# ramanathanlab/distllm

Measured on NVIDIA H100. Metric: embedded chunks/sec @512-tok, higher is better.
Workload: dtype bf16

## Files before the change

### distllm_b200/csrc/attention.cuh

```cuda
#pragma once

#include "common.cuh"

namespace b2e {

constexpr int AT_KC = 64;
constexpr float AT_MASKED = -3.0e38f;

template <int D, int V>
struct AtCfg {
  static constexpr int COLS = D < 64 ? D : 64;
  static constexpr int ROW_BYTES = 2 * COLS;
  static constexpr int BOX = 64 * ROW_BYTES;
  static constexpr int NB = D / COLS;
  static constexpr int NWG = (V & 64) ? 4 : 2;
  static constexpr int QT = 64 * NWG;
  static constexpr int THREADS = 128 * NWG + (NWG == 4 ? 128 : 32);
  static constexpr int CONSUMER_REGS = 112, PRODUCER_REGS = 24;
  static constexpr int STAGES = D == 128 ? 3 : 4;
  static constexpr int Q_BYTES = NWG * NB * BOX;
  static constexpr int STAGE_BYTES = 2 * NB * BOX;
  static_assert(D == 32 || D == 64 || D == 128, "head_dim");
  static constexpr int BAR = Q_BYTES + STAGES * STAGE_BYTES;
  static constexpr int SMEM_BYTES = BAR + 256 + 1024;
  static_assert(SMEM_BYTES <= 232448, "shared memory");
};

__device__ long long* g_att_clock = nullptr;

__device__ __forceinline__ float poly_exp2(float x) {
  x = fmaxf(x, -126.0f);
  const float n = rintf(x);
  const float f = x - n;
  float p = fmaf(f, 9.6181291e-3f, 5.5504109e-2f);
  p = fmaf(f, p, 2.4022651e-1f);
  p = fmaf(f, p, 6.9314718e-1f);
  p = fmaf(f, p, 1.0f);
  return __int_as_float(__float_as_int(p) + (static_cast<int>(n) << 23));
}

template <int ROW_BYTES>
__device__ __forceinline__ uint64_t at_box_desc(uint32_t saddr) {
  if constexpr (ROW_BYTES == 128) return make_smem_desc_sw128(saddr);
  else return make_smem_desc_sw64(saddr);
}

__global__ void attn_prep_kernel(const int64_t* __restrict__ mask, float* __restrict__ bias,
                                 int* __restrict__ kv_chunks, int* __restrict__ plain_chunks, int B, int S,
                                 int S_pad) {
  const int b = blockIdx.x * (blockDim.x >> 5) + (threadIdx.x >> 5);
  if (b >= B) return;
  const int lane = threadIdx.x & 31;
  int last = 0;
  int first_off = S_pad;
  for (int j = lane; j < S_pad; j += 32) {
    float v = -INFINITY;
    bool on = false;
    if (j < S) {
      on = mask[static_cast<size_t>(b) * S + j] != 0;
      v = on ? 0.0f : AT_MASKED;
      if (on) last = j + 1;
    }
    if (!on) first_off = min(first_off, j);
    bias[static_cast<size_t>(b) * S_pad + j] = v;
  }
#pragma unroll
  for (int o = 16; o > 0; o >>= 1) {
    last = max(last, __shfl_xor_sync(0xffffffffu, last, o));
    first_off = min(first_off, __shfl_xor_sync(0xffffffffu, first_off, o));
  }
  if (lane == 0) {
    kv_chunks[b] = last > 0 ? (last + AT_KC - 1) / AT_KC : S_pad / AT_KC;
    plain_chunks[b] = first_off / AT_KC;
  }
}

template <int D, int MODE, int V>
__global__ void __launch_bounds__(AtCfg<D, V>::THREADS, 1)
attention_kernel(const __grid_constant__ CUtensorMap tm, const __grid_constant__ CUtensorMap tm_ctx,
                 const float* __restrict__ bias, const int* __restrict__ kv_chunks,
                 const int* __restrict__ plain_chunks, int B, int S, int S_pad, int heads, int kv_heads, int window,
                 float scale_log2e, const int* __restrict__ seq_cu, const int* __restrict__ seq_len,
                 h16* __restrict__ ctx) {
  using Cfg = AtCfg<D, V>;
  constexpr int NB = Cfg::NB;
  constexpr int COLS = Cfg::COLS, BOX = Cfg::BOX, RB = Cfg::ROW_BYTES;
  constexpr int NWG = Cfg::NWG;
  constexpr int POLY = (V >> 2) & 3;
  constexpr bool EPI_ROLE = (V & 128) != 0;
  constexpr bool STAMPS = (V & 256) != 0;
  static_assert(MODE == 0 || (V & ~(64 | 128)) == 0, "windowed / causal attention: warpgroups and epilogue role only");
  const int h = blockIdx.x % heads;
  const int b = (blockIdx.x / heads) % B;
  const int tile = static_cast<int>(gridDim.x / (heads * B)) - 1 - static_cast<int>(blockIdx.x / (heads * B));
  const int row0 = seq_cu != nullptr ? __ldg(seq_cu + b) : b * S;
  const int len = seq_len != nullptr ? __ldg(seq_len + b) : S;
  const int q0 = tile * Cfg::QT;
  if (q0 >= len) return;
  const int kvc = __ldg(kv_chunks + b);
  const int np = (V & 1) ? __ldg(plain_chunks + b) : 0;
  int lo = 0, hi = kvc;
  if (MODE == 1) {
    lo = max(0, q0 - window) / AT_KC;
    hi = min(kvc, (q0 + Cfg::QT - 1 + window) / AT_KC + 1);
  } else if (MODE == 2) {
    lo = window > 0 ? max(0, q0 - window + 1) / AT_KC : 0;
    hi = min(kvc, (q0 + Cfg::QT - 1) / AT_KC + 1);
  }
  if (lo >= hi) lo = hi - 1;

  extern __shared__ uint8_t smem_raw[];
  const uint32_t sb = (smem_u32(smem_raw) + 1023u) & ~1023u;
  const uint32_t q_bar = sb + Cfg::BAR;
  const uint32_t full_bar = q_bar + 8;
  const uint32_t empty_bar = full_bar + 8u * Cfg::STAGES;
  const uint32_t out_bar = empty_bar + 8u * Cfg::STAGES;
  const int warp = threadIdx.x >> 5;
  const int kvh = h / (heads / kv_heads);
  const int qcol = h * D, kcol = (heads + kvh) * D, vcol = (heads + kv_heads + kvh) * D;

  if (threadIdx.x == 0) {
    mbar_init(q_bar, 1);
    for (int s = 0; s < Cfg::STAGES; ++s) {
      mbar_init(full_bar + 8u * s, 1);
      mbar_init(empty_bar + 8u * s, NWG);
    }
    for (int w = 0; w < NWG; ++w) mbar_init(out_bar + 8u * w, 1);
    mbar_fence_init();
  }
  __syncthreads();

  if (warp >= 4 * NWG) {
    if constexpr (NWG == 4) asm volatile("setmaxnreg.dec.sync.aligned.u32 %0;" ::"n"(Cfg::PRODUCER_REGS));
    if (warp == 4 * NWG && elect_one()) {
      tma_prefetch_desc(&tm);
      mbar_expect_tx(q_bar, Cfg::Q_BYTES);
#pragma unroll
      for (int w = 0; w < NWG; ++w)
#pragma unroll
        for (int x = 0; x < NB; ++x)
          tma_load_2d(sb + (w * NB + x) * BOX, &tm, q_bar, qcol + COLS * x, row0 + q0 + 64 * w);
      int stage = 0;
      uint32_t phase = 0;
      for (int c = lo; c < hi; ++c) {
        mbar_wait(empty_bar + 8u * stage, phase ^ 1u);
        const uint32_t fb = full_bar + 8u * stage;
        const uint32_t dst = sb + Cfg::Q_BYTES + stage * Cfg::STAGE_BYTES;
        mbar_expect_tx(fb, Cfg::STAGE_BYTES);
#pragma unroll
        for (int x = 0; x < NB; ++x) {
          tma_load_2d(dst + x * BOX, &tm, fb, kcol + COLS * x, row0 + c * AT_KC);
          tma_load_2d(dst + (NB + x) * BOX, &tm, fb, vcol + COLS * x, row0 + c * AT_KC);
        }
        if (++stage == Cfg::STAGES) { stage = 0; phase ^= 1u; }
      }
      if constexpr (EPI_ROLE) {
        for (int w = 0; w < NWG; ++w) {
          mbar_wait(out_bar + 8u * w, 0);
          if (q0 + 64 * w + 64 > len) continue;
#pragma unroll
          for (int x = 0; x < NB; ++x)
            tma_store_2d(&tm_ctx, sb + (w * NB + x) * BOX, h * D + COLS * x, row0 + q0 + 64 * w);
        }
        tma_store_commit();
        tma_store_wait_all();
      }
    }
    return;
  }

  if constexpr (NWG == 4) asm volatile("setmaxnreg.inc.sync.aligned.u32 %0;" ::"n"(Cfg::CONSUMER_REGS));
  const int wg = warp >> 2;
  const int t = threadIdx.x & 127;
  const int quad = t & 3;
  const int qr = q0 + 64 * wg + 16 * (t >> 5) + ((t & 31) >> 2);
  const float* brow = bias + static_cast<size_t>(b) * S_pad;
  const uint32_t q_addr = sb + wg * NB * BOX;
  long long* clk = nullptr;
  int n_stamp = 0;
  if (STAMPS && blockIdx.x == 0 && threadIdx.x == 0) clk = g_att_clock;

  constexpr int OG = COLS / 8;
  float o[NB][4 * OG];
#pragma unroll
  for (int x = 0; x < NB; ++x)
#pragma unroll
    for (int i = 0; i < 4 * OG; ++i) o[x][i] = 0.0f;
  float m[2] = {-INFINITY, -INFINITY}, l[2] = {0.0f, 0.0f};

  mbar_wait(q_bar, 0);
  int stage = 0;
  uint32_t phase = 0;
  for (int c = lo; c < hi; ++c) {
    mbar_wait(full_bar + 8u * stage, phase);
    const uint32_t k_addr = sb + Cfg::Q_BYTES + stage * Cfg::STAGE_BYTES;
    const uint32_t v_addr = k_addr + NB * BOX;
    float s[32];
#pragma unroll
    for (int i = 0; i < 32; ++i) s[i] = 0.0f;
    wgmma_fence();
    constexpr int KB = COLS / 16;
#pragma unroll
    for (int kk = 0; kk < D / 16; ++kk)
      wgmma_64x64_ss<0>(s, at_box_desc<RB>(q_addr + (kk / KB) * BOX) + 2u * (kk % KB),
                        at_box_desc<RB>(k_addr + (kk / KB) * BOX) + 2u * (kk % KB), kk != 0);
    wgmma_commit();
    wgmma_wait<0>();
    reg_fence(s);
    if (STAMPS && clk != nullptr && n_stamp < 256) {
      clk[n_stamp] = clock64();
      clk[256 + n_stamp++] = 2 * c + 1;
    }

    const int kbase = c * AT_KC + 2 * quad;
    const bool plain = MODE == 0 && (V & 1) && c < np;
#pragma unroll
    for (int j = 0; j < 8; ++j) {
      const float2 bz = plain ? make_float2(0.0f, 0.0f) : *reinterpret_cast<const float2*>(brow + kbase + 8 * j);
#pragma unroll
      for (int e = 0; e < 4; ++e) {
        const int key = kbase + 8 * j + (e & 1);
        const int q = qr + 8 * (e >> 1);
        float x = fmaf(s[4 * j + e], scale_log2e, (e & 1) ? bz.y : bz.x);
        if (MODE == 1 && abs(q - key) > window) x = AT_MASKED;
        if (MODE == 2 && (key > q || (window > 0 && q - key >= window))) x = AT_MASKED;
        s[4 * j + e] = x;
      }
    }
    float alpha[2];
#pragma unroll
    for (int hf = 0; hf < 2; ++hf) {
      float mx = m[hf];
#pragma unroll
      for (int j = 0; j < 8; ++j) mx = fmaxf(mx, fmaxf(s[4 * j + 2 * hf], s[4 * j + 2 * hf + 1]));
      mx = fmaxf(mx, __shfl_xor_sync(0xffffffffu, mx, 1));
      mx = fmaxf(mx, __shfl_xor_sync(0xffffffffu, mx, 2));
      alpha[hf] = fast_exp2(m[hf] - mx);
      m[hf] = mx;
    }
    uint32_t p[4][4];
    float rs[2] = {0.0f, 0.0f};
#pragma unroll
    for (int j = 0; j < 8; ++j) {
#pragma unroll
      for (int hf = 0; hf < 2; ++hf) {
        const float x0 = s[4 * j + 2 * hf] - m[hf], x1 = s[4 * j + 2 * hf + 1] - m[hf];
        const int k0 = (2 * (j & 1) + hf) * 2;
        const float p0 = (k0 % 4) < POLY ? poly_exp2(x0) : fast_exp2(x0);
        const float p1 = ((k0 + 1) % 4) < POLY ? poly_exp2(x1) : fast_exp2(x1);
        rs[hf] += p0 + p1;
        p[j >> 1][(j & 1) * 2 + hf] = pack_h16x2(p0, p1);
      }
    }
#pragma unroll
    for (int hf = 0; hf < 2; ++hf) l[hf] = l[hf] * alpha[hf] + rs[hf];
#pragma unroll
    for (int x = 0; x < NB; ++x)
#pragma unroll
      for (int j = 0; j < OG; ++j) {
        o[x][4 * j + 0] *= alpha[0];
        o[x][4 * j + 1] *= alpha[0];
        o[x][4 * j + 2] *= alpha[1];
        o[x][4 * j + 3] *= alpha[1];
      }

#pragma unroll
    for (int x = 0; x < NB; ++x) reg_fence(o[x]);
    wgmma_fence();
#pragma unroll
    for (int kc = 0; kc < 4; ++kc)
#pragma unroll
      for (int x = 0; x < NB; ++x) {
        if constexpr (COLS == 64) wgmma_64x64_rs_tb(o[x], p[kc], make_smem_desc_sw128(v_addr + x * BOX + kc * 16 * 128));
        else wgmma_64x32_rs_tb(o[x], p[kc], make_smem_desc_sw64(v_addr + x * BOX + kc * 16 * 64));
      }
    wgmma_commit();
    wgmma_wait<0>();
#pragma unroll
    for (int x = 0; x < NB; ++x) reg_fence(o[x]);
    if (STAMPS && clk != nullptr && n_stamp < 256) {
      clk[n_stamp] = clock64();
      clk[256 + n_stamp++] = 2 * c + 2;
    }
    if (t == 0) mbar_arrive(empty_bar + 8u * stage);
    if (++stage == Cfg::STAGES) { stage = 0; phase ^= 1u; }
  }

  const bool staged = EPI_ROLE && q0 + 64 * wg + 64 <= len;
#pragma unroll
  for (int hf = 0; hf < 2; ++hf) {
    float tot = l[hf];
    tot += __shfl_xor_sync(0xffffffffu, tot, 1);
    tot += __shfl_xor_sync(0xffffffffu, tot, 2);
    const float inv = 1.0f / tot;
    const int q = qr + 8 * hf;
    if (staged) {
      const int r = q - q0 - 64 * wg;
      const int swz = RB == 128 ? (r & 7) : ((r >> 1) & 3);
#pragma unroll
      for (int x = 0; x < NB; ++x)
#pragma unroll
        for (int j = 0; j < OG; ++j) {
          const uint32_t off = r * RB + ((j ^ swz) << 4) + 4 * quad;
          *reinterpret_cast<uint32_t*>(smem_raw + (q_addr - smem_u32(smem_raw)) + x * BOX + off) =
              pack_h16x2(o[x][4 * j + 2 * hf] * inv, o[x][4 * j + 2 * hf + 1] * inv);
        }
      continue;
    }
    if (q >= len) continue;
    h16* orow = ctx + static_cast<size_t>(row0 + q) * (heads * D) + h * D + 2 * quad;
#pragma unroll
    for (int x = 0; x < NB; ++x)
#pragma unroll
      for (int j = 0; j < OG; ++j)
        *reinterpret_cast<uint32_t*>(orow + COLS * x + 8 * j) =
            pack_h16x2(o[x][4 * j + 2 * hf] * inv, o[x][4 * j + 2 * hf + 1] * inv);
  }
  if constexpr (EPI_ROLE) {
    fence_proxy_async_smem();
    asm volatile("bar.sync %0, 128;" ::"r"(1 + wg) : "memory");
    if (t == 0) mbar_arrive(out_bar + 8u * wg);
  }
}

}
```

### distllm_b200/csrc/b2e_api.cu

```cuda
#include "../../include/b2e.h"
#include "../../include/b2e_debug.h"

#include <cuda.h>
#include <cuda_runtime.h>

#include <cstdarg>
#include <cstdio>
#include <cstdlib>
#include <cstring>
#include <string>
#include <utility>
#include <vector>

#include "attention.cuh"
#include "binsearch.cuh"
#include "common.cuh"
#include "gemm.cuh"
#include "mistral_ops.cuh"
#include "pack.cuh"
#include "rowops.cuh"
#include "topk.cuh"
#include "topk_tc.cuh"

using namespace b2e;
// ... 102 lines not shown
  info->ok = true;
  return B2E_OK;
}

int current_device_info(DeviceInfo* info) {
  int dev = 0;
  if (cudaGetDevice(&dev) != cudaSuccess) {
    cudaGetLastError();
    return fail(B2E_ERR_NO_DEVICE, "no CUDA device visible; libb2e has no CPU fallback");
  }
  static DeviceInfo cache[64];
  if (dev < 64 && cache[dev].ok) {
    *info = cache[dev];
    return B2E_OK;
  }
  int rc = device_info(dev, info);
  if (rc == B2E_OK && dev < 64) cache[dev] = *info;
  return rc;
}

template <typename Kern>
int ensure_smem_attr(Kern kern, int bytes) {
  static std::vector<std::pair<const void*, int>> done;
  int dev = 0;
  CUDA_TRY(cudaGetDevice(&dev));
  const void* key = reinterpret_cast<const void*>(kern);
  for (const auto& d : done)
    if (d.first == key && d.second == dev) return B2E_OK;
  CUDA_TRY(cudaFuncSetAttribute(kern, cudaFuncAttributeMaxDynamicSharedMemorySize, bytes));
  done.emplace_back(key, dev);
  return B2E_OK;
}

int check_gemm_shape(int M, int N, int K) {
  if (M <= 0 || N <= 0 || K <= 0) return fail(B2E_ERR_INVALID, "gemm: empty shape %dx%dx%d", M, N, K);
  if (N % 128 != 0) return fail(B2E_ERR_INVALID, "gemm: N=%d must be a multiple of 128", N);
  if (K % 64 != 0) return fail(B2E_ERR_INVALID, "gemm: K=%d must be a multiple of 64", K);
  return B2E_OK;
}

bool g_gemm_profiling = false;

template <int EPI>
int launch_gemm_epi(const CUtensorMap& ta, const CUtensorMap& tb, void* out, const float* bias,
                    const h16* resid, int M, int N, int K, cudaStream_t st, const int* m_dev) {
  auto kern = gemm_h16_wgmma_kernel<EPI>;
  if constexpr (EPI == EPI_BIAS)
    if (g_gemm_profiling) kern = gemm_h16_wgmma_kernel<EPI, true>;
  int rc = ensure_smem_attr(kern, GEMM_SMEM_BYTES);
  if (rc) return rc;
  DeviceInfo dev;
  if ((rc = current_device_info(&dev))) return rc;
  const long long tiles = (long long)(N / GEMM_BN) * ((M + GEMM_BM - 1) / GEMM_BM);
  if (tiles > 0x7fffffffLL) return fail(B2E_ERR_INVALID, "gemm: %lld output tiles exceed one grid", tiles);
  CUtensorMap tm_out;
  if ((rc = make_tmap_h16(&tm_out, out, M, epi_is_glu(EPI) ? N / 2 : N, GEMM_BM))) return rc;
  const unsigned grid = (unsigned)(tiles < dev.sms ? tiles : dev.sms);
  kern<<<grid, GEMM_THREADS, GEMM_SMEM_BYTES, st>>>(ta, tb, tm_out, static_cast<h16*>(out), bias, resid, M, N, K,
                                                    m_dev);
  CUDA_TRY(cudaGetLastError());
  return B2E_OK;
}

int launch_gemm(const CUtensorMap& ta, const CUtensorMap& tb, void* out, const float* bias,
                const void* resid, int M, int N, int K, int epi, cudaStream_t st, const int* m_dev = nullptr) {
  const h16* r = static_cast<const h16*>(resid);
  switch (epi) {
    case B2E_EPI_BIAS: return launch_gemm_epi<EPI_BIAS>(ta, tb, out, bias, r, M, N, K, st, m_dev);
    case B2E_EPI_BIAS_GELU: return launch_gemm_epi<EPI_BIAS_GELU>(ta, tb, out, bias, r, M, N, K, st, m_dev);
    case B2E_EPI_BIAS_RESID: return launch_gemm_epi<EPI_BIAS_RESID>(ta, tb, out, bias, r, M, N, K, st, m_dev);
    case B2E_EPI_SWIGLU: return launch_gemm_epi<EPI_SWIGLU>(ta, tb, out, bias, r, M, N, K, st, m_dev);
    case B2E_EPI_GEGLU: return launch_gemm_epi<EPI_GEGLU>(ta, tb, out, bias, r, M, N, K, st, m_dev);
  }
  return fail(B2E_ERR_INVALID, "unknown epilogue %d", epi);
}

struct AttnScratch {
  float* bias = nullptr;
  int* kv_chunks = nullptr;
  int* plain_chunks = nullptr;
  size_t cap_bias = 0, cap_b = 0;
  uint64_t gen = 0;
  int device = -1;
  int ensure(int B, int S_pad) {
    int dev = 0;
    CUDA_TRY(cudaGetDevice(&dev));
    if (dev != device) {
      release();
      device = dev;
      ++gen;
    }
    if ((size_t)B * S_pad > cap_bias || (size_t)B > cap_b) ++gen;
    if ((size_t)B * S_pad > cap_bias) {
      cudaFree(bias);
      bias = nullptr;
      cap_bias = 0;
      CUDA_TRY(cudaMalloc(&bias, sizeof(float) * (size_t)B * S_pad));
      cap_bias = (size_t)B * S_pad;
    }
    if ((size_t)B > cap_b) {
      cudaFree(kv_chunks); cudaFree(plain_chunks);
      kv_chunks = plain_chunks = nullptr;
      cap_b = 0;
      CUDA_TRY(cudaMalloc(&kv_chunks, sizeof(int) * B));
      CUDA_TRY(cudaMalloc(&plain_chunks, sizeof(int) * B));
      cap_b = B;
    }
    return B2E_OK;
  }
  void release() {
    cudaFree(bias); cudaFree(kv_chunks); cudaFree(plain_chunks);
    bias = nullptr; kv_chunks = plain_chunks = nullptr; cap_bias = cap_b = 0;
  }
};

inline int attn_s_pad(int S) { return (S + AT_KC - 1) / AT_KC * AT_KC; }

int attention_prepare(AttnScratch& sc, const int64_t* mask, int B, int S, cudaStream_t st) {
  int rc;
  const int S_pad = attn_s_pad(S);
  if ((rc = sc.ensure(B, S_pad))) return rc;
  attn_prep_kernel<<<(B + 7) / 8, 256, 0, st>>>(mask, sc.bias, sc.kv_chunks, sc.plain_chunks, B, S, S_pad);
  CUDA_TRY(cudaGetLastError());
  return B2E_OK;
}

struct SeqLayout {
  const int* cu = nullptr;
  const int* len = nullptr;
  const int* t_real = nullptr;
  const int* tok_src = nullptr;
};

template <int D, int MODE, int V>
int launch_attention_kernel(const CUtensorMap& tm, const AttnScratch& sc, void* ctx, int B, int S, int heads,
                            int kv_heads, int window, cudaStream_t st, const SeqLayout& lay) {
  using Cfg = AtCfg<D, V>;
  auto kern = attention_kernel<D, MODE, V>;
  int rc = ensure_smem_attr(kern, Cfg::SMEM_BYTES);
  if (rc) return rc;
  CUtensorMap tm_ctx = {};
  if ((V & 128) && (rc = make_tmap_h16(&tm_ctx, ctx, (uint64_t)B * S, (uint64_t)heads * D, 64, Cfg::COLS))) return rc;
  const float scale_log2e = 1.4426950408889634f / sqrtf(static_cast<float>(D));
  const long long ctas = (long long)heads * B * ((S + Cfg::QT - 1) / Cfg::QT);
  if (ctas > 0x7fffffffLL)
    return fail(B2E_ERR_INVALID, "attention: %lld CTAs (heads=%d B=%d S=%d) exceed one grid", ctas, heads, B, S);
  kern<<<(unsigned)ctas, Cfg::THREADS, Cfg::SMEM_BYTES, st>>>(tm, tm_ctx, sc.bias, sc.kv_chunks, sc.plain_chunks, B, S,
                                                    attn_s_pad(S), heads, kv_heads, window, scale_log2e, lay.cu,
                                                    lay.len, static_cast<h16*>(ctx));
  CUDA_TRY(cudaGetLastError());
  return B2E_OK;
}

constexpr int AT_DEFAULT_VARIANT = 193;
int g_att3_variant = -1;
inline int att3_variant() {
  if (g_att3_variant < 0) {
    const char* e = getenv("B2E_ATT3");
    g_att3_variant = e ? atoi(e) : AT_DEFAULT_VARIANT;
  }
  return g_att3_variant;
}

int launch_attention(const CUtensorMap& tkv, const AttnScratch& sc, void* ctx, int B, int S, int heads,
                     cudaStream_t st, int window = 0, const SeqLayout& lay = SeqLayout()) {
  const int v = att3_variant();
#define B2E_ATT(MODE, V) launch_attention_kernel<64, MODE, V>(tkv, sc, ctx, B, S, heads, heads, window, st, lay)
  if (window > 0) {
    switch (v & 192) {
      case 0: return B2E_ATT(1, 0);
      case 64: return B2E_ATT(1, 64);
      case 128: return B2E_ATT(1, 128);
      case 192: return B2E_ATT(1, 192);
    }
    return fail(B2E_ERR_INVALID, "windowed attention: variant %d has no instantiation (bits 6-7 of the variant pick "
                "0, 64, 128 or 192)", v);
  }
  switch (v) {
    case 0: return B2E_ATT(0, 0);
    case 1: return B2E_ATT(0, 1);
    case 5: return B2E_ATT(0, 5);
    case 64: return B2E_ATT(0, 64);
    case 65: return B2E_ATT(0, 65);
    case 69: return B2E_ATT(0, 69);
    case 193: return B2E_ATT(0, 193);
    case 261: return B2E_ATT(0, 261);
    case 321: return B2E_ATT(0, 321);
  }
#undef B2E_ATT
  return fail(B2E_ERR_INVALID, "attention variant %d is not instantiated (0,1,5,64,65,69,193,261,321)", v);
}

int launch_attention_causal_d128(const void* qkv, AttnScratch& sc, void* ctx, int B, int S, int heads,
                                 int kv_heads, int window, cudaStream_t st, const SeqLayout& lay = SeqLayout()) {
  CUtensorMap tm;
  const int rc = make_tmap_h16(&tm, qkv, (uint64_t)B * S, (uint64_t)(heads + 2 * kv_heads) * 128, AT_KC);
  if (rc) return rc;
  return launch_attention_kernel<128, 2, 0>(tm, sc, ctx, B, S, heads, kv_heads, window, st, lay);
}

constexpr int AT_D32_VARIANT = 1;

int launch_attention_bidir(const CUtensorMap& tqkv, const AttnScratch& sc, void* ctx, int B, int S, int heads,
                           int head_dim, cudaStream_t st, const SeqLayout& lay = SeqLayout()) {
  if (head_dim == 32)
    return launch_attention_kernel<32, 0, AT_D32_VARIANT>(tqkv, sc, ctx, B, S, heads, heads, 0, st, lay);
  return launch_attention(tqkv, sc, ctx, B, S, heads, st, 0, lay);
}

#define DISPATCH_H(H, CALL)                                         \
  switch (H) {                                                      \
    case 256: { constexpr int HW = 256; CALL; break; }              \
    case 384: { constexpr int HW = 384; CALL; break; }              \
    case 512: { constexpr int HW = 512; CALL; break; }              \
    case 640: { constexpr int HW = 640; CALL; break; }              \
    case 768: { constexpr int HW = 768; CALL; break; }              \
    case 1024: { constexpr int HW = 1024; CALL; break; }            \
    case 1280: { constexpr int HW = 1280; CALL; break; }            \
    case 2048: { constexpr int HW = 2048; CALL; break; }            \
    case 2560: { constexpr int HW = 2560; CALL; break; }            \
    case 4096: { constexpr int HW = 4096; CALL; break; }            \
    default: return fail(B2E_ERR_INVALID, "hidden size %d not supported (need 256*{1,2,3,4,5,8,10,16}, 384 or 640)", (H)); \
  }

inline int row_blocks(int rows) { return (rows + ROW_WARPS - 1) / ROW_WARPS; }

int check_h(int H) {
  if (H == 384 || H == 640) return B2E_OK;
  if (H % 256 != 0) return fail(B2E_ERR_INVALID, "hidden size %d must be a multiple of 256, or 384 or 640", H);
  switch (H / 256) {
    case 1: case 2: case 3: case 4: case 5: case 8: case 10: case 16: return B2E_OK;
  }
  return fail(B2E_ERR_UNSUPPORTED, "hidden size %d not supported (built: 256 x {1,2,3,4,5,8,10,16}, 384, 640)", H);
}

struct PoolScratch {
  int* seq_len = nullptr;
  int* kill = nullptr;
  int* idx = nullptr;
  float* w = nullptr;
  float* count = nullptr;
  float* part = nullptr;
  size_t cap_b = 0, cap_s = 0, cap_bs = 0, cap_part = 0;
  int device = -1;
  uint64_t gen = 0;

  int ensure(int B, int S, size_t part_elems) {
    int dev = 0;
    CUDA_TRY(cudaGetDevice(&dev));
    if (dev != device) {
      release();
      device = dev;
      ++gen;
    }
    if ((size_t)B > cap_b || (size_t)S > cap_s || (size_t)B * S > cap_bs || part_elems > cap_part) ++gen;
    if ((size_t)B > cap_b) {
      cudaFree(seq_len); cudaFree(idx); cudaFree(count);
      seq_len = idx = nullptr;
      count = nullptr;
      cap_b = 0;
      CUDA_TRY(cudaMalloc(&seq_len, sizeof(int) * B));
      CUDA_TRY(cudaMalloc(&idx, sizeof(int) * B));
      CUDA_TRY(cudaMalloc(&count, sizeof(float) * B));
      cap_b = B;
    }
    if ((size_t)S > cap_s) {
      cudaFree(kill);
      kill = nullptr;
      cap_s = 0;
      CUDA_TRY(cudaMalloc(&kill, sizeof(int) * S));
      cap_s = S;
    }
    if ((size_t)B * S > cap_bs) {
      cudaFree(w);
      w = nullptr;
      cap_bs = 0;
      CUDA_TRY(cudaMalloc(&w, sizeof(float) * (size_t)B * S));
      cap_bs = (size_t)B * S;
    }
    if (part_elems > cap_part) {
      cudaFree(part);
      part = nullptr;
      cap_part = 0;
      CUDA_TRY(cudaMalloc(&part, sizeof(float) * part_elems));
      cap_part = part_elems;
    }
    return B2E_OK;
  }
  void release() {
    cudaFree(seq_len); cudaFree(kill); cudaFree(idx); cudaFree(w); cudaFree(count); cudaFree(part);
    seq_len = kill = idx = nullptr; w = count = part = nullptr;
    cap_b = cap_s = cap_bs = cap_part = 0;
  }
};

inline int pool_nsplit(int S) {
  int n = (S + 63) / 64;
  return n < 1 ? 1 : (n > 16 ? 16 : n);
}

int launch_pool_weights(PoolScratch& ps, int64_t* mask, int B, int S, int pool_kind, int mutate,
                        cudaStream_t st) {
  seq_len_kernel<<<(B + 7) / 8, 256, 0, st>>>(mask, ps.seq_len, B, S);
  CUDA_TRY(cudaMemsetAsync(ps.kill, 0, sizeof(int) * S, st));
  kill_columns_kernel<<<(B + 255) / 256, 256, 0, st>>>(ps.seq_len, ps.kill, B, S);
  pool_weights_kernel<<<(B + 7) / 8, 256, 0, st>>>(mask, ps.seq_len, ps.kill, ps.w, ps.count, B, S,
                                                    pool_kind == B2E_POOL_MEAN_REF ? 1 : 0, mutate);
  CUDA_TRY(cudaGetLastError());
  return B2E_OK;
}

int launch_finalize(PoolScratch& ps, float* out, int B, int H, int nsplit, int l2, int round_mode,
                    cudaStream_t st) {
  pool_finalize_kernel<<<B, 256, (H + 32) * sizeof(float), st>>>(ps.part, ps.count, out, H, nsplit,
                                                                 l2, round_mode);
  CUDA_TRY(cudaGetLastError());
  return B2E_OK;
}

struct DeviceGuard {
  int prev = -1;
  DeviceGuard() {
    if (cudaGetDevice(&prev) != cudaSuccess) {
      cudaGetLastError();
      prev = -1;
    }
  }
  ~DeviceGuard() {
    if (prev >= 0) cudaSetDevice(prev);
  }
};

thread_local PoolScratch g_pool_scratch;
thread_local AttnScratch g_attn_scratch;

}

struct B2EEncoder {
  B2EModelDesc desc;
  int full_layers = 0;
  std::vector<const void*> w;
  int device = 0;
  int sms = 0;
// ... 1343 lines not shown
```

Baseline: 3170.

## Add persistent bidirectional attention kernel with double-buffered Q and TMA output stores

Adds a persistent attention kernel for head_dim 64 that loops over (head, batch, q-tile) work items on a grid sized to SM occupancy. Q is double-buffered so the producer can load the next tile's Q and K/V while consumers finish the current one, and the output is staged in the Q buffer and written with TMA stores. The default variant switches from 193 to 577, a 4-warpgroup persistent configuration. This is meant to cut per-CTA launch, prologue and epilogue cost and keep the pipeline full across tiles, at the price of doubling Q shared memory and a more complex barrier protocol.

```diff
diff --git a/distllm_b200/csrc/attention.cuh b/distllm_b200/csrc/attention.cuh
--- a/distllm_b200/csrc/attention.cuh
+++ b/distllm_b200/csrc/attention.cuh
@@ -19,9 +19,10 @@
   static constexpr int CONSUMER_REGS = 112, PRODUCER_REGS = 24;
   static constexpr int STAGES = D == 128 ? 3 : 4;
   static constexpr int Q_BYTES = NWG * NB * BOX;
+  static constexpr int Q_BUFS = (V & 512) ? 2 : 1;
   static constexpr int STAGE_BYTES = 2 * NB * BOX;
   static_assert(D == 32 || D == 64 || D == 128, "head_dim");
-  static constexpr int BAR = Q_BYTES + STAGES * STAGE_BYTES;
+  static constexpr int BAR = Q_BUFS * Q_BYTES + STAGES * STAGE_BYTES;
   static constexpr int SMEM_BYTES = BAR + 256 + 1024;
   static_assert(SMEM_BYTES <= 232448, "shared memory");
 };
@@ -323,4 +324,282 @@
   }
 }
 
-}
+
+__device__ __forceinline__ void at_softmax_chunk(float (&s)[32], float (&m)[2], float (&l)[2], float (&alpha)[2],
+                                                 const float* brow, int c, bool plain, int quad, float scale_log2e) {
+  const int kbase = c * AT_KC + 2 * quad;
+#pragma unroll
+  for (int j = 0; j < 8; ++j) {
+    const float2 bz = plain ? make_float2(0.0f, 0.0f) : *reinterpret_cast<const float2*>(brow + kbase + 8 * j);
+#pragma unroll
+    for (int e = 0; e < 4; ++e) s[4 * j + e] = fmaf(s[4 * j + e], scale_log2e, (e & 1) ? bz.y : bz.x);
+  }
+#pragma unroll
+  for (int hf = 0; hf < 2; ++hf) {
+    float mx = m[hf];
+#pragma unroll
+    for (int j = 0; j < 8; ++j) mx = fmaxf(mx, fmaxf(s[4 * j + 2 * hf], s[4 * j + 2 * hf + 1]));
+    mx = fmaxf(mx, __shfl_xor_sync(0xffffffffu, mx, 1));
+    mx = fmaxf(mx, __shfl_xor_sync(0xffffffffu, mx, 2));
+    alpha[hf] = fast_exp2(m[hf] - mx);
+    m[hf] = mx;
+  }
+  float rs[2] = {0.0f, 0.0f};
+#pragma unroll
+  for (int j = 0; j < 8; ++j) {
+#pragma unroll
+    for (int hf = 0; hf < 2; ++hf) {
+      const float x0 = s[4 * j + 2 * hf] - m[hf], x1 = s[4 * j + 2 * hf + 1] - m[hf];
+      const float p0 = fast_exp2(x0), p1 = fast_exp2(x1);
+      rs[hf] += p0 + p1;
+      s[4 * j + 2 * hf] = p0;
+      s[4 * j + 2 * hf + 1] = p1;
+    }
+  }
+#pragma unroll
+  for (int hf = 0; hf < 2; ++hf) l[hf] = l[hf] * alpha[hf] + rs[hf];
+}
+
+struct AtItem {
+  int h, b, q0, row0, len;
+};
+__device__ __forceinline__ AtItem at_item(int it, int heads, int B, int tiles, int qt, int S, const int* seq_cu,
+                                          const int* seq_len) {
+  AtItem r;
+  r.h = it % heads;
+  r.b = (it / heads) % B;
+  r.q0 = (tiles - 1 - it / (heads * B)) * qt;
+  r.row0 = seq_cu != nullptr ? __ldg(seq_cu + r.b) : r.b * S;
+  r.len = seq_len != nullptr ? __ldg(seq_len + r.b) : S;
+  return r;
+}
+
+template <int V>
+__global__ void __launch_bounds__(AtCfg<64, V>::THREADS, 1)
+attention_persistent_kernel(const __grid_constant__ CUtensorMap tm, const __grid_constant__ CUtensorMap tm_ctx,
+                            const float* __restrict__ bias, const int* __restrict__ kv_chunks,
+                            const int* __restrict__ plain_chunks, int B, int S, int S_pad, int heads, int tiles,
+                            float scale_log2e, const int* __restrict__ seq_cu, const int* __restrict__ seq_len,
+                            h16* __restrict__ ctx) {
+  using Cfg = AtCfg<64, V>;
+  static_assert((V & 512) && (V & ~(512 | 64 | 1)) == 0, "persistent kernel: bits 0, 6 and 9 only");
+  constexpr int BOX = Cfg::BOX, NWG = Cfg::NWG, QT = Cfg::QT;
+  constexpr bool PIPELINED = NWG == 2;
+  const int items = heads * B * tiles;
+
+  extern __shared__ uint8_t smem_raw[];
+  const uint32_t sb = (smem_u32(smem_raw) + 1023u) & ~1023u;
+  const uint32_t kv0 = sb + 2 * Cfg::Q_BYTES;
+  const uint32_t q_full = sb + Cfg::BAR;
+  const uint32_t q_empty = q_full + 16;
+  const uint32_t full_bar = q_empty + 16;
+  const uint32_t empty_bar = full_bar + 8u * Cfg::STAGES;
+  const int warp = threadIdx.x >> 5;
+
+  if (threadIdx.x == 0) {
+    for (int i = 0; i < 2; ++i) {
+      mbar_init(q_full + 8u * i, 1);
+      mbar_init(q_empty + 8u * i, NWG);
+    }
+    for (int s = 0; s < Cfg::STAGES; ++s) {
+      mbar_init(full_bar + 8u * s, 1);
+      mbar_init(empty_bar + 8u * s, NWG);
+    }
+    mbar_fence_init();
+  }
+  __syncthreads();
+
+  if (warp >= 4 * NWG) {
+    if constexpr (NWG == 4) asm volatile("setmaxnreg.dec.sync.aligned.u32 %0;" ::"n"(Cfg::PRODUCER_REGS));
+    if (warp == 4 * NWG && elect_one()) {
+      tma_prefetch_desc(&tm);
+      int stage = 0, n = 0;
+      uint32_t phase = 0;
+      for (int it = blockIdx.x; it < items; it += gridDim.x) {
+        const AtItem w = at_item(it, heads, B, tiles, QT, S, seq_cu, seq_len);
+        if (w.q0 >= w.len) continue;
+        const int kvc = __ldg(kv_chunks + w.b);
+        const int qb = n & 1;
+        mbar_wait(q_empty + 8u * qb, ((n >> 1) & 1) ^ 1u);
+        mbar_expect_tx(q_full + 8u * qb, Cfg::Q_BYTES);
+#pragma unroll
+        for (int g = 0; g < NWG; ++g)
+          tma_load_2d(sb + qb * Cfg::Q_BYTES + g * BOX, &tm, q_full + 8u * qb, w.h * 64, w.row0 + w.q0 + 64 * g);
+        const int kcol = (heads + w.h) * 64, vcol = (2 * heads + w.h) * 64;
+        for (int c = 0; c < kvc; ++c) {
+          mbar_wait(empty_bar + 8u * stage, phase ^ 1u);
+          const uint32_t fb = full_bar + 8u * stage;
+          const uint32_t dst = kv0 + stage * Cfg::STAGE_BYTES;
+          mbar_expect_tx(fb, Cfg::STAGE_BYTES);
+          tma_load_2d(dst, &tm, fb, kcol, w.row0 + c * AT_KC);
+          tma_load_2d(dst + BOX, &tm, fb, vcol, w.row0 + c * AT_KC);
+          if (++stage == Cfg::STAGES) { stage = 0; phase ^= 1u; }
+        }
+        ++n;
+      }
+    }
+    return;
+  }
+
+  if constexpr (NWG == 4) asm volatile("setmaxnreg.inc.sync.aligned.u32 %0;" ::"n"(Cfg::CONSUMER_REGS));
+  const int wg = warp >> 2;
+  const int t = threadIdx.x & 127;
+  const int quad = t & 3;
+  const int r_lo = 16 * (t >> 5) + ((t & 31) >> 2);
+  int stage = 0, n = 0;
+  uint32_t phase = 0;
+  int pend = -1;
+
+  auto issue_s = [&](float (&s)[32], uint32_t q_addr, int st) {
+    const uint32_t k_addr = kv0 + st * Cfg::STAGE_BYTES;
+#pragma unroll
+    for (int kk = 0; kk < 4; ++kk)
+      wgmma_64x64_ss<0>(s, make_smem_desc_sw128(q_addr) + 2u * kk, make_smem_desc_sw128(k_addr) + 2u * kk, kk != 0);
+    wgmma_commit();
+  };
+  auto issue_pv = [&](float (&o)[32], const uint32_t (&p)[4][4], int st) {
+    const uint32_t v_addr = kv0 + st * Cfg::STAGE_BYTES + BOX;
+#pragma unroll
+    for (int kc = 0; kc < 4; ++kc) wgmma_64x64_rs_tb(o, p[kc], make_smem_desc_sw128(v_addr + kc * 16 * 128));
+    wgmma_commit();
+  };
+  auto pack = [&](uint32_t (&p)[4][4], const float (&s)[32]) {
+#pragma unroll
+    for (int j = 0; j < 8; ++j)
+#pragma unroll
+      for (int hf = 0; hf < 2; ++hf) p[j >> 1][(j & 1) * 2 + hf] = pack_h16x2(s[4 * j + 2 * hf], s[4 * j + 2 * hf + 1]);
+  };
+
+  for (int it = blockIdx.x; it < items; it += gridDim.x) {
+    const AtItem w = at_item(it, heads, B, tiles, QT, S, seq_cu, seq_len);
+    if (w.q0 >= w.len) continue;
+    const int kvc = __ldg(kv_chunks + w.b);
+    const int np = (V & 1) ? __ldg(plain_chunks + w.b) : 0;
+    const float* brow = bias + static_cast<size_t>(w.b) * S_pad;
+    const int qb = n & 1;
+    const uint32_t q_addr = sb + qb * Cfg::Q_BYTES + wg * BOX;
+
+    float o[32], s[32];
+#pragma unroll
+    for (int i = 0; i < 32; ++i) o[i] = 0.0f;
+    float m[2] = {-INFINITY, -INFINITY}, l[2] = {0.0f, 0.0f}, alpha[2];
+    uint32_t p[4][4];
+
+    mbar_wait(q_full + 8u * qb, (n >> 1) & 1);
+    if constexpr (!PIPELINED) {
+      for (int c = 0; c < kvc; ++c) {
+        mbar_wait(full_bar + 8u * stage, phase);
+        wgmma_fence();
+        issue_s(s, q_addr, stage);
+        if (c == 0 && t == 0 && pend >= 0) {
+          tma_store_wait_read<0>();
+          mbar_arrive(q_empty + 8u * pend);
+          pend = -1;
+        }
+        wgmma_wait<0>();
+        reg_fence(s);
+        at_softmax_chunk(s, m, l, alpha, brow, c, (V & 1) && c < np, quad, scale_log2e);
+#pragma unroll
+        for (int j = 0; j < 8; ++j) {
+          o[4 * j + 0] *= alpha[0];
+          o[4 * j + 1] *= alpha[0];
+          o[4 * j + 2] *= alpha[1];
+          o[4 * j + 3] *= alpha[1];
+        }
+        pack(p, s);
+        reg_fence(o);
+        wgmma_fence();
+        issue_pv(o, p, stage);
+        wgmma_wait<0>();
+        reg_fence(o);
+        if (t == 0) mbar_arrive(empty_bar + 8u * stage);
+        if (++stage == Cfg::STAGES) { stage = 0; phase ^= 1u; }
+      }
+    } else {
+      mbar_wait(full_bar + 8u * stage, phase);
+      wgmma_fence();
+      issue_s(s, q_addr, stage);
+      if (t == 0 && pend >= 0) {
+        tma_store_wait_read<0>();
+        mbar_arrive(q_empty + 8u * pend);
+        pend = -1;
+      }
+      wgmma_wait<0>();
+      reg_fence(s);
+      at_softmax_chunk(s, m, l, alpha, brow, 0, (V & 1) && 0 < np, quad, scale_log2e);
+      pack(p, s);
+      int pstage = stage;
+      if (++stage == Cfg::STAGES) { stage = 0; phase ^= 1u; }
+
+      for (int c = 1; c < kvc; ++c) {
+        mbar_wait(full_bar + 8u * stage, phase);
+        reg_fence(o);
+        wgmma_fence();
+        issue_s(s, q_addr, stage);
+        issue_pv(o, p, pstage);
+        wgmma_wait<1>();
+        reg_fence(s);
+        at_softmax_chunk(s, m, l, alpha, brow, c, (V & 1) && c < np, quad, scale_log2e);
+        wgmma_wait<0>();
+        reg_fence(o);
+  #pragma unroll
+        for (int j = 0; j < 8; ++j) {
+          o[4 * j + 0] *= alpha[0];
+          o[4 * j + 1] *= alpha[0];
+          o[4 * j + 2] *= alpha[1];
+          o[4 * j + 3] *= alpha[1];
+        }
+        pack(p, s);
+        if (t == 0) mbar_arrive(empty_bar + 8u * pstage);
+        pstage = stage;
+        if (++stage == Cfg::STAGES) { stage = 0; phase ^= 1u; }
+      }
+      reg_fence(o);
+      wgmma_fence();
+      issue_pv(o, p, pstage);
+      wgmma_wait<0>();
+      reg_fence(o);
+      if (t == 0) mbar_arrive(empty_bar + 8u * pstage);
+    }
+
+    const AtItem e = at_item(it, heads, B, tiles, QT, S, seq_cu, seq_len);
+    const bool staged = e.q0 + 64 * wg + 64 <= e.len;
+    uint8_t* qbox = smem_raw + (q_addr - smem_u32(smem_raw));
+#pragma unroll
+    for (int hf = 0; hf < 2; ++hf) {
+      float tot = l[hf];
+      tot += __shfl_xor_sync(0xffffffffu, tot, 1);
+      tot += __shfl_xor_sync(0xffffffffu, tot, 2);
+      const float inv = 1.0f / tot;
+      const int r = r_lo + 8 * hf;
+      if (staged) {
+#pragma unroll
+        for (int j = 0; j < 8; ++j)
+          *reinterpret_cast<uint32_t*>(qbox + r * 128 + ((j ^ (r & 7)) << 4) + 4 * quad) =
+              pack_h16x2(o[4 * j + 2 * hf] * inv, o[4 * j + 2 * hf + 1] * inv);
+        continue;
+      }
+      const int q = e.q0 + 64 * wg + r;
+      if (q >= e.len) continue;
+      h16* orow = ctx + static_cast<size_t>(e.row0 + q) * (heads * 64) + e.h * 64 + 2 * quad;
+#pragma unroll
+      for (int j = 0; j < 8; ++j)
+        *reinterpret_cast<uint32_t*>(orow + 8 * j) = pack_h16x2(o[4 * j + 2 * hf] * inv, o[4 * j + 2 * hf + 1] * inv);
+    }
+    if (staged) {
+      fence_proxy_async_smem();
+      named_bar_sync(1 + wg, 128);
+      if (t == 0) {
+        tma_store_2d(&tm_ctx, q_addr, e.h * 64, e.row0 + e.q0 + 64 * wg);
+        tma_store_commit();
+        pend = qb;
+      }
+    } else if (t == 0) {
+      mbar_arrive(q_empty + 8u * qb);
+    }
+    ++n;
+  }
+  if (t == 0 && pend >= 0) tma_store_wait_all();
+}
+
+}
diff --git a/distllm_b200/csrc/b2e_api.cu b/distllm_b200/csrc/b2e_api.cu
--- a/distllm_b200/csrc/b2e_api.cu
+++ b/distllm_b200/csrc/b2e_api.cu
@@ -278,7 +278,33 @@
   return B2E_OK;
 }
 
-constexpr int AT_DEFAULT_VARIANT = 193;
+template <int V>
+int launch_attention_persistent(const CUtensorMap& tm, const AttnScratch& sc, void* ctx, int B, int S, int heads,
+                                cudaStream_t st, const SeqLayout& lay) {
+  using Cfg = AtCfg<64, V>;
+  auto kern = attention_persistent_kernel<V>;
+  int rc = ensure_smem_attr(kern, Cfg::SMEM_BYTES);
+  if (rc) return rc;
+  DeviceInfo dev;
+  if ((rc = current_device_info(&dev))) return rc;
+  static int per_sm = 0;
+  if (per_sm == 0) CUDA_TRY(cudaOccupancyMaxActiveBlocksPerMultiprocessor(&per_sm, kern, Cfg::THREADS, Cfg::SMEM_BYTES));
+  if (per_sm == 0) return fail(B2E_ERR_CUDA, "attention: the persistent kernel does not fit on an SM");
+  CUtensorMap tm_ctx;
+  if ((rc = make_tmap_h16(&tm_ctx, ctx, (uint64_t)B * S, (uint64_t)heads * 64, 64))) return rc;
+  const int tiles = (S + Cfg::QT - 1) / Cfg::QT;
+  const long long items = (long long)heads * B * tiles;
+  if (items > 0x7fffffffLL)
+    return fail(B2E_ERR_INVALID, "attention: %lld items (heads=%d B=%d S=%d) exceed one grid", items, heads, B, S);
+  const long long slots = (long long)dev.sms * per_sm;
+  kern<<<(unsigned)(items < slots ? items : slots), Cfg::THREADS, Cfg::SMEM_BYTES, st>>>(
+      tm, tm_ctx, sc.bias, sc.kv_chunks, sc.plain_chunks, B, S, attn_s_pad(S), heads, tiles,
+      1.4426950408889634f / 8.0f, lay.cu, lay.len, static_cast<h16*>(ctx));
+  CUDA_TRY(cudaGetLastError());
+  return B2E_OK;
+}
+
+constexpr int AT_DEFAULT_VARIANT = 577;
 int g_att3_variant = -1;
 inline int att3_variant() {
   if (g_att3_variant < 0) {
@@ -293,7 +319,7 @@
   const int v = att3_variant();
 #define B2E_ATT(MODE, V) launch_attention_kernel<64, MODE, V>(tkv, sc, ctx, B, S, heads, heads, window, st, lay)
   if (window > 0) {
-    switch (v & 192) {
+    switch ((v & 512) ? 192 : (v & 192)) {
       case 0: return B2E_ATT(1, 0);
       case 64: return B2E_ATT(1, 64);
       case 128: return B2E_ATT(1, 128);
@@ -312,9 +338,11 @@
     case 193: return B2E_ATT(0, 193);
     case 261: return B2E_ATT(0, 261);
     case 321: return B2E_ATT(0, 321);
+    case 513: return launch_attention_persistent<513>(tkv, sc, ctx, B, S, heads, st, lay);
+    case 577: return launch_attention_persistent<577>(tkv, sc, ctx, B, S, heads, st, lay);
   }
 #undef B2E_ATT
-  return fail(B2E_ERR_INVALID, "attention variant %d is not instantiated (0,1,5,64,65,69,193,261,321)", v);
+  return fail(B2E_ERR_INVALID, "attention variant %d is not instantiated (0,1,5,64,65,69,193,261,321,513,577)", v);
 }
 
 int launch_attention_causal_d128(const void* qkv, AttnScratch& sc, void* ctx, int B, int S, int heads,
```

Measured after the change: 3200 (median of 6 runs). No clear change (+1.0%).

## Add lazy-rescale softmax attention variant and make it default

Applied to the files above, without the earlier changes.

Adds a LAZY attention path (variant bit 512, default now 705) for head_dim 64. The running max is only raised when a new tile's max exceeds it by more than a threshold, so the O accumulator is rescaled only when some lane moved. The path also folds the scale into the exponent FMA for unmasked chunks and issues the first QK wgmma with scale-d=0 so the accumulator zeroing is skipped. This cuts per-tile FMA, max and exp work, at the cost of exponent headroom: probabilities can reach 2^8 before packing to 16-bit.

```diff
diff --git a/distllm_b200/csrc/attention.cuh b/distllm_b200/csrc/attention.cuh
--- a/distllm_b200/csrc/attention.cuh
+++ b/distllm_b200/csrc/attention.cuh
@@ -6,6 +6,7 @@
 
 constexpr int AT_KC = 64;
 constexpr float AT_MASKED = -3.0e38f;
+constexpr float AT_RESCALE_LOG2 = 8.0f;
 
 template <int D, int V>
 struct AtCfg {
@@ -45,6 +46,65 @@
   else return make_smem_desc_sw64(saddr);
 }
 
+__device__ __forceinline__ void at_issue_qk64(float (&s)[32], uint32_t q_addr, uint32_t k_addr) {
+  asm volatile(
+      "{\n.reg .pred p;\nsetp.ne.b32 p, 0, 0;\n"
+      "wgmma.mma_async.sync.aligned.m64n64k16.f32." B2E_WGMMA_AB " "
+      "{%0,%1,%2,%3,%4,%5,%6,%7,%8,%9,%10,%11,%12,%13,%14,%15,"
+      "%16,%17,%18,%19,%20,%21,%22,%23,%24,%25,%26,%27,%28,%29,%30,%31}, %32, %33, p, 1, 1, 0, 0;\n}\n"
+      : "=f"(s[0]), "=f"(s[1]), "=f"(s[2]), "=f"(s[3]), "=f"(s[4]), "=f"(s[5]), "=f"(s[6]), "=f"(s[7]),
+        "=f"(s[8]), "=f"(s[9]), "=f"(s[10]), "=f"(s[11]), "=f"(s[12]), "=f"(s[13]), "=f"(s[14]), "=f"(s[15]),
+        "=f"(s[16]), "=f"(s[17]), "=f"(s[18]), "=f"(s[19]), "=f"(s[20]), "=f"(s[21]), "=f"(s[22]), "=f"(s[23]),
+        "=f"(s[24]), "=f"(s[25]), "=f"(s[26]), "=f"(s[27]), "=f"(s[28]), "=f"(s[29]), "=f"(s[30]), "=f"(s[31])
+      : "l"(make_smem_desc_sw128(q_addr)), "l"(make_smem_desc_sw128(k_addr)));
+#pragma unroll
+  for (int kk = 1; kk < 4; ++kk)
+    wgmma_64x64_ss<0>(s, make_smem_desc_sw128(q_addr) + 2u * kk, make_smem_desc_sw128(k_addr) + 2u * kk, 1);
+}
+template <bool PLAIN>
+__device__ __forceinline__ bool at_softmax_lazy(float (&s)[32], const float* __restrict__ bk, float c, float (&m)[2],
+                                                float (&l)[2], float (&alpha)[2], uint32_t (&p)[4][4]) {
+  if constexpr (!PLAIN) {
+#pragma unroll
+    for (int j = 0; j < 8; ++j) {
+      const float2 bz = *reinterpret_cast<const float2*>(bk + 8 * j);
+#pragma unroll
+      for (int e = 0; e < 4; ++e) s[4 * j + e] = fmaf(s[4 * j + e], c, (e & 1) ? bz.y : bz.x);
+    }
+  }
+  bool moved = false;
+  float neg_m[2];
+#pragma unroll
+  for (int hf = 0; hf < 2; ++hf) {
+    float mx = fmaxf(s[2 * hf], s[2 * hf + 1]);
+#pragma unroll
+    for (int j = 1; j < 8; ++j) mx = fmaxf(mx, fmaxf(s[4 * j + 2 * hf], s[4 * j + 2 * hf + 1]));
+    mx = fmaxf(mx, __shfl_xor_sync(0xffffffffu, mx, 1));
+    mx = fmaxf(mx, __shfl_xor_sync(0xffffffffu, mx, 2));
+    if (PLAIN) mx *= c;
+    const bool up = mx > m[hf] + AT_RESCALE_LOG2;
+    alpha[hf] = up ? fast_exp2(m[hf] - mx) : 1.0f;
+    if (up) m[hf] = mx;
+    moved |= up;
+    neg_m[hf] = -m[hf];
+  }
+  float rs[2] = {0.0f, 0.0f};
+#pragma unroll
+  for (int j = 0; j < 8; ++j) {
+#pragma unroll
+    for (int hf = 0; hf < 2; ++hf) {
+      const float x0 = s[4 * j + 2 * hf], x1 = s[4 * j + 2 * hf + 1];
+      const float p0 = fast_exp2(PLAIN ? fmaf(x0, c, neg_m[hf]) : x0 + neg_m[hf]);
+      const float p1 = fast_exp2(PLAIN ? fmaf(x1, c, neg_m[hf]) : x1 + neg_m[hf]);
+      rs[hf] += p0 + p1;
+      p[j >> 1][(j & 1) * 2 + hf] = pack_h16x2(p0, p1);
+    }
+  }
+#pragma unroll
+  for (int hf = 0; hf < 2; ++hf) l[hf] = fmaf(l[hf], alpha[hf], rs[hf]);
+  return __any_sync(0xffffffffu, moved);
+}
+
 __global__ void attn_prep_kernel(const int64_t* __restrict__ mask, float* __restrict__ bias,
                                  int* __restrict__ kv_chunks, int* __restrict__ plain_chunks, int B, int S,
                                  int S_pad) {
@@ -89,7 +149,9 @@
   constexpr int POLY = (V >> 2) & 3;
   constexpr bool EPI_ROLE = (V & 128) != 0;
   constexpr bool STAMPS = (V & 256) != 0;
+  constexpr bool LAZY = (V & 512) != 0;
   static_assert(MODE == 0 || (V & ~(64 | 128)) == 0, "windowed / causal attention: warpgroups and epilogue role only");
+  static_assert(!LAZY || (D == 64 && (V & (12 | 256)) == 0), "cheaper softmax: head_dim 64, MUFU exponentials, no stamps");
   const int h = blockIdx.x % heads;
   const int b = (blockIdx.x / heads) % B;
   const int tile = static_cast<int>(gridDim.x / (heads * B)) - 1 - static_cast<int>(blockIdx.x / (heads * B));
@@ -191,19 +253,26 @@
   mbar_wait(q_bar, 0);
   int stage = 0;
   uint32_t phase = 0;
+  if constexpr (LAZY) m[0] = m[1] = AT_MASKED;
   for (int c = lo; c < hi; ++c) {
     mbar_wait(full_bar + 8u * stage, phase);
     const uint32_t k_addr = sb + Cfg::Q_BYTES + stage * Cfg::STAGE_BYTES;
     const uint32_t v_addr = k_addr + NB * BOX;
     float s[32];
-#pragma unroll
-    for (int i = 0; i < 32; ++i) s[i] = 0.0f;
+    if constexpr (!LAZY) {
+#pragma unroll
+      for (int i = 0; i < 32; ++i) s[i] = 0.0f;
+    }
     wgmma_fence();
     constexpr int KB = COLS / 16;
-#pragma unroll
-    for (int kk = 0; kk < D / 16; ++kk)
-      wgmma_64x64_ss<0>(s, at_box_desc<RB>(q_addr + (kk / KB) * BOX) + 2u * (kk % KB),
-                        at_box_desc<RB>(k_addr + (kk / KB) * BOX) + 2u * (kk % KB), kk != 0);
+    if constexpr (LAZY) {
+      at_issue_qk64(s, q_addr, k_addr);
+    } else {
+#pragma unroll
+      for (int kk = 0; kk < D / 16; ++kk)
+        wgmma_64x64_ss<0>(s, at_box_desc<RB>(q_addr + (kk / KB) * BOX) + 2u * (kk % KB),
+                          at_box_desc<RB>(k_addr + (kk / KB) * BOX) + 2u * (kk % KB), kk != 0);
+    }
     wgmma_commit();
     wgmma_wait<0>();
     reg_fence(s);
@@ -212,6 +281,22 @@
       clk[256 + n_stamp++] = 2 * c + 1;
     }
 
+    uint32_t p[4][4];
+    if constexpr (LAZY) {
+      const float* bk = brow + c * AT_KC + 2 * quad;
+      float alpha[2];
+      const bool moved = (V & 1) && c < np ? at_softmax_lazy<true>(s, bk, scale_log2e, m, l, alpha, p)
+                                           : at_softmax_lazy<false>(s, bk, scale_log2e, m, l, alpha, p);
+      if (moved) {
+#pragma unroll
+        for (int j = 0; j < 8; ++j) {
+          o[0][4 * j + 0] *= alpha[0];
+          o[0][4 * j + 1] *= alpha[0];
+          o[0][4 * j + 2] *= alpha[1];
+          o[0][4 * j + 3] *= alpha[1];
+        }
+      }
+    } else {
     const int kbase = c * AT_KC + 2 * quad;
     const bool plain = MODE == 0 && (V & 1) && c < np;
 #pragma unroll
@@ -238,7 +323,6 @@
       alpha[hf] = fast_exp2(m[hf] - mx);
       m[hf] = mx;
     }
-    uint32_t p[4][4];
     float rs[2] = {0.0f, 0.0f};
 #pragma unroll
     for (int j = 0; j < 8; ++j) {
@@ -264,6 +348,7 @@
         o[x][4 * j + 3] *= alpha[1];
       }
 
+    }
 #pragma unroll
     for (int x = 0; x < NB; ++x) reg_fence(o[x]);
     wgmma_fence();
diff --git a/distllm_b200/csrc/b2e_api.cu b/distllm_b200/csrc/b2e_api.cu
--- a/distllm_b200/csrc/b2e_api.cu
+++ b/distllm_b200/csrc/b2e_api.cu
@@ -278,7 +278,7 @@
   return B2E_OK;
 }
 
-constexpr int AT_DEFAULT_VARIANT = 193;
+constexpr int AT_DEFAULT_VARIANT = 705;
 int g_att3_variant = -1;
 inline int att3_variant() {
   if (g_att3_variant < 0) {
@@ -312,9 +312,10 @@
     case 193: return B2E_ATT(0, 193);
     case 261: return B2E_ATT(0, 261);
     case 321: return B2E_ATT(0, 321);
+    case 705: return B2E_ATT(0, 705);
   }
 #undef B2E_ATT
-  return fail(B2E_ERR_INVALID, "attention variant %d is not instantiated (0,1,5,64,65,69,193,261,321)", v);
+  return fail(B2E_ERR_INVALID, "attention variant %d is not instantiated (0,1,5,64,65,69,193,261,321,705)", v);
 }
 
 int launch_attention_causal_d128(const void* qkv, AttnScratch& sc, void* ctx, int B, int S, int heads,
```

New measurement: 3183 before, 3247 after, median of 6. 2.0% higher.
